# adobe/3D-FM-GAN

Measured on AMD Instinct MI355X. Metric: (photo,render) pairs/sec, higher is better.
Workload: dtype f32; 1 GPU; pairs1024: cfg4 shard: E_Tsr+E_W+E_W_Plus(18 styles) on 256^2 -> co-mod -> Generator(1024) forward, fp32, B=8/GPU; pairs_per_gpu=8, global_pairs=8, image_size=1024, parallelism=replicas x1 (batch-sharded, no collective), launch=eager, ranks=1, full=False

## Files before the change

3d-fm-gan_amd/csrc/modconv_fwd.hip:

```cpp
#include <type_traits>
#include "common.h"
#include <cstdio>
#include <cstdlib>

namespace {

typedef unsigned u32x2 __attribute__((ext_vector_type(2)));

template <int SIZE, typename RSRC>
__device__ __forceinline__ void dma_to_lds(RSRC rsrc, float* lds, unsigned voff, unsigned soff) {
#if defined(__HIP_DEVICE_COMPILE__)
  typedef __attribute__((address_space(3))) void* lds_void_ptr;
  __builtin_amdgcn_raw_ptr_buffer_load_lds(rsrc, (lds_void_ptr)lds, SIZE, voff, soff, 0, 0);
#endif
}

__device__ __forceinline__ const float* uniform_ptr(const float* q) {
  const unsigned long long v = (unsigned long long)q;
  const unsigned lo = __builtin_amdgcn_readfirstlane((unsigned)v), hi = __builtin_amdgcn_readfirstlane((unsigned)(v >> 32));
  return (const float*)(((unsigned long long)hi << 32) | lo);
}
__device__ __forceinline__ unsigned uniform_u32(unsigned v) { return __builtin_amdgcn_readfirstlane(v); }

struct MCParams {
  const float* in; const float* wt; const float* style; const float* demod; float* out;
  int batch, cin, cout, h, w, oh, ow;
  long long out_plane_stride; int out_row_stride;
  struct Seg {
    int m_off, n_off, gh, gw;
    int th, nb, tw_log2;
    int tiles_x, tiles_y, tiles_b;
    unsigned block_end;
    int wide;
  } seg[3];
  int nseg, o_tiles;
  int ksplit, cin_per_split;
  float* ws;
  const float* noise; const float* noise_weight; const float* bias;
  int noise_batch, fuse_act; float alpha, act_scale;
  const float* rgb_wmod;
  const float* rgb_bias; const float* rgb_skip; float* rgb_out;
  int rgb_c;
  int lds_buf_floats, lds_patch_floats;
  int lds_style_floats;
  int debug;
  unsigned long long* dbg_clock;
  int exp_flags;
};

#ifdef FMGAN_EXPERIMENTS
#define MC_DEBUG(p) ((p).debug)
#define MC_CLOCK(p) ((p).dbg_clock)
#define MC_FLAGS(p) ((p).exp_flags)
#else
#define MC_DEBUG(p) 0
#define MC_CLOCK(p) false
#define MC_FLAGS(p) 0
#endif

constexpr int MC_KC = 8;

__device__ __forceinline__ float mc_epilogue(float v, const MCParams& p, float nw, int b, int o, int pix) {
  if (p.demod) v *= p.demod[(long long)b * p.cout + o];
  if (p.fuse_act) {
    const float n = p.noise ? p.noise[(long long)(p.noise_batch == 1 ? 0 : b) * p.oh * p.ow + pix] : 0.f;
    const float bv = p.bias ? p.bias[o] : 0.f;
    v = __fadd_rn(__fadd_rn(v, __fmul_rn(nw, n)), bv);
    v = (v > 0.f ? v : v * p.alpha) * p.act_scale;
  }
  return v;
}

template <int MODE_, int RM_, int RNP_, int WM_, int WN_, int MINB_, int KC_, int PIPE_>
struct TileShape {
  static constexpr int MODE = MODE_, RM = RM_, RNP = RNP_, WM = WM_, WN = WN_, MINB = MINB_, KC = KC_, PIPE = PIPE_;
  static constexpr int BM = 32 * RM * WM, BN = 32 * RNP * WN;
};
struct Plain128x128Reg         : TileShape<   0,  2,   2,  2,  2,    2, MC_KC,    0> {};
struct Plain128x128DmaKc4      : TileShape<   0,  2,   2,  2,  2,    3,     4,    1> {};
struct Plain128x256DmaKc4      : TileShape<   0,  4,   2,  1,  4,    2,     4,    1> {};
struct Plain64x128Reg          : TileShape<   0,  2,   1,  1,  4,    3, MC_KC,    0> {};
struct Plain64x128Dma          : TileShape<   0,  2,   1,  1,  4,    3,     8,    1> {};
struct Plain64x256DmaKc4       : TileShape<   0,  2,   2,  1,  4,    3,     4,    1> {};
struct Plain32x128Reg          : TileShape<   0,  1,   1,  1,  4,    4, MC_KC,    0> {};
struct Plain32x128Dma          : TileShape<   0,  1,   1,  1,  4,    4,     8,    1> {};
struct Plain32x256DmaKc4R128   : TileShape<   0,  1,   2,  1,  4,    4,     4,    1> {};
struct Stride2x128x128Reg      : TileShape<   2,  2,   2,  2,  2,    2, MC_KC,    0> {};
struct Stride2x64x128Reg       : TileShape<   2,  2,   1,  1,  4,    2, MC_KC,    0> {};
struct Stride2x32x128Reg       : TileShape<   2,  1,   1,  1,  4,    2, MC_KC,    0> {};
struct Transposed64x128Reg     : TileShape<   1,  2,   1,  1,  4,    2, MC_KC,    0> {};
struct Transposed64x128Dma     : TileShape<   1,  2,   1,  1,  4,    2,     8,    1> {};
struct Transposed32x128Reg     : TileShape<   1,  1,   1,  1,  4,    3, MC_KC,    0> {};
struct Transposed32x128DmaR128 : TileShape<   1,  1,   1,  1,  4,    4,     8,    1> {};
#ifdef FMGAN_EXPERIMENTS
struct Plain32x256Dma          : TileShape<   0,  1,   2,  1,  4,    3,     8,    1> {};
struct Plain32x256DmaKc4R96    : TileShape<   0,  1,   2,  1,  4,    5,     4,    1> {};
struct Transposed32x256Dma     : TileShape<   1,  1,   2,  1,  4,    2,     8,    1> {};
struct Transposed32x128DmaR170 : TileShape<   1,  1,   1,  1,  4,    3,     8,    1> {};
#endif

template <class Tile, bool RGB>
__global__ __launch_bounds__(256, Tile::MINB) void modconv_mfma_f32(const MCParams p) {
  constexpr int MODE = Tile::MODE, RM = Tile::RM, RNP = Tile::RNP, WM = Tile::WM, WN = Tile::WN, KC = Tile::KC, PIPE = Tile::PIPE;
  static_assert(!RGB || MODE == 0, "the RGB epilogue belongs to the plain conv");
  static_assert(PIPE == 1 || KC == MC_KC, "the register pipeline is built for 8-channel chunks");
  constexpr int BM = Tile::BM;
  constexpr int NPH = MODE == 1 ? 4 : 1;
  static_assert(WM * WN == 4, "4 waves per block");
  extern __shared__ float smem[];
  float* Ws = smem;
  float* Xs = smem + KC * 9 * BM;

  const int tid = threadIdx.x, lane = tid & 63, wave = __builtin_amdgcn_readfirstlane(tid >> 6);
  const int wm = wave / WN, wn = wave % WN;
  const int l31 = lane & 31, khalf = lane >> 5;
  unsigned long long clk0 = 0, rt0 = 0;
  if (MC_CLOCK(p)) { clk0 = __builtin_readcyclecounter(); rt0 = wall_clock64(); }
  if (MC_FLAGS(p) & 1) __builtin_amdgcn_s_setprio(3);

  unsigned lb = xcd_remap(blockIdx.x, gridDim.x);
  int si = 0;
  while (si + 1 < p.nseg && lb >= p.seg[si].block_end) ++si;
  if (si > 0) lb -= p.seg[si - 1].block_end;
  const unsigned tapmask = (MODE == 1 && p.nseg == 3) ? (si == 0 ? 0x1C0u : (si == 1 ? 0x124u : 0x1FFu)) : 0x1FFu;
  const int seg_th = p.seg[si].th, seg_nb = p.seg[si].nb, tw_log2 = p.seg[si].tw_log2;
  const int seg_m_end = p.seg[si].m_off + p.seg[si].gh, seg_n_end = p.seg[si].n_off + p.seg[si].gw;
  constexpr int SP = MODE == 2 ? 2 : 1;
  constexpr int ORG = MODE == 2 ? 0 : 1;
  const bool wide = PIPE == 1 && SP == 1 && p.seg[si].wide != 0;
  const int XORG = wide ? 4 : ORG;
  const int TW = 1 << tw_log2, PWP = wide ? TW + 8 : SP * (TW - 1) + 3;
  const int o_tile = lb % p.o_tiles;
  unsigned pt = lb / p.o_tiles;
  const int tx_i = pt % p.seg[si].tiles_x; pt /= p.seg[si].tiles_x;
  const int ty_i = pt % p.seg[si].tiles_y;
  const int tb_i = pt / p.seg[si].tiles_y;
  const int ks = blockIdx.y;
  const int o0 = o_tile * BM, b0 = tb_i * seg_nb;
  const int x0 = p.seg[si].n_off + tx_i * TW, y0 = p.seg[si].m_off + ty_i * seg_th;
  const int PH = SP * (seg_th - 1) + 3;
  const int plane = PH * PWP;
  const int samp = KC * plane;

  int pbase[RNP], pos_b[RNP], pos_y[RNP], pos_x[RNP];
#pragma unroll
  for (int g = 0; g < RNP; ++g) {
    const int pos = (wn * RNP + g) * 32 + l31;
    const int tx = pos & (TW - 1), r = pos >> tw_log2;
    const int ty = r % seg_th, nbi = r / seg_th;
    pbase[g] = min(nbi, seg_nb - 1) * samp + SP * ty * PWP + SP * tx + (XORG - ORG);
    pos_b[g] = nbi < seg_nb ? b0 + nbi : p.batch; pos_y[g] = y0 + ty; pos_x[g] = x0 + tx;
  }

  f32x16 acc[RM][RNP][NPH];
#pragma unroll
  for (int a = 0; a < RM; ++a)
#pragma unroll
    for (int b = 0; b < RNP; ++b)
#pragma unroll
      for (int c = 0; c < NPH; ++c)
#pragma unroll
        for (int r = 0; r < 16; ++r) acc[a][b][c][r] = 0.f;

  const bool wvec = (p.cout & 3) == 0;
  const int i_begin = ks * p.cin_per_split;
  const int i_end = min(p.cin, i_begin + p.cin_per_split);
  const int hw = p.h * p.w;

  constexpr int BNP = 32 * RNP * WN;
  constexpr int NU = ((SP * (BNP / 32 - 1) + 3) * (SP * 31 + 3) + 255) / 256;
  constexpr int NWV = (KC * 9 * (BM / 4) + 255) / 256;
  const int spatial = seg_nb * plane;
  const float* in_b0 = uniform_ptr(p.in + (long long)b0 * p.cin * hw);
  const float* style_b0 = uniform_ptr(p.style + (long long)b0 * p.cin);
  const bool epi_lds = PIPE == 1 && seg_nb == 1 && p.ksplit == 1;
  float* Es = smem + 2 * p.lds_buf_floats;
  float epi_v = 0.f;
  if constexpr (PIPE == 1) {
    if (epi_lds && tid < 2 * BM) {
      const bool isd = tid >= BM;
      const int oc = min(o0 + (isd ? tid - BM : tid), p.cout - 1);
      epi_v = isd ? 1.f : 0.f;
      if (isd) { if (p.demod) epi_v = p.demod[(long long)min(b0, p.batch - 1) * p.cout + oc]; }
      else if (MODE == 0 && p.fuse_act && p.bias) epi_v = p.bias[oc];
    }
  }
  int gofs[NU], lofs[NU], sofs[NU]; bool inb[NU];
#pragma unroll
  for (int u = 0; u < NU; ++u) {
    const int q = tid + 256 * u;
    const int c = q % PWP;
    int t = q / PWP;
    const int r = t % PH, nbi = t / PH;
    const int b = b0 + nbi, y = SP * y0 + r - ORG, x = SP * x0 + c - ORG;
    inb[u] = q < spatial && b < p.batch && y >= 0 && y < p.h && x >= 0 && x < p.w;
    gofs[u] = inb[u] ? (nbi * p.cin * p.h + y) * p.w + x : 0;
    sofs[u] = nbi * p.cin;
    lofs[u] = q < spatial ? nbi * samp + r * PWP + c : -1;
  }
  float xv[NU][KC];
  f32x4 wv[NWV];
  constexpr long long PARK = 0xFFFFFFF0LL;
  const bool fastw = wvec && o0 + BM <= p.cout && (long long)p.cin * 9 * p.cout * 4 < PARK;
  const bool fastx = (long long)min(seg_nb, p.batch - b0) * p.cin * hw * 4 < PARK;
  const unsigned w_bytes = uniform_u32((unsigned)((long long)p.cin * 9 * p.cout * 4));
  const unsigned x_bytes = uniform_u32((unsigned)((long long)min(seg_nb, p.batch - b0) * p.cin * hw * 4));
  const auto rsrc_w = __builtin_amdgcn_make_buffer_rsrc(const_cast<float*>(p.wt), 0, w_bytes, 0x00020000);
  const auto rsrc_x = __builtin_amdgcn_make_buffer_rsrc(const_cast<float*>(in_b0), 0, x_bytes, 0x00020000);
  unsigned wofs[NWV], xofs[NU];
#pragma unroll
  for (int j = 0; j < NWV; ++j) {
    const int idx = tid + 256 * j;
    const int row = idx / (BM / 4), c4 = idx % (BM / 4);
    wofs[j] = idx < KC * 9 * (BM / 4) ? (unsigned)((row * p.cout + o0 + c4 * 4) * 4) : 0xFFFFFFF0u;
  }
#pragma unroll
  for (int u = 0; u < NU; ++u) xofs[u] = inb[u] ? (unsigned)gofs[u] * 4u : 0xFFFFFFF0u;
  auto issue = [&](int i0) {
    if (fastw && i0 + KC <= i_end) {
      const unsigned soff = (unsigned)(i0 * 9 * p.cout * 4);
#pragma unroll
      for (int j = 0; j < NWV; ++j) {
        const auto t = __builtin_amdgcn_raw_buffer_load_b128(rsrc_w, wofs[j], soff, 0);
        wv[j] = __builtin_bit_cast(f32x4, t);
      }
    } else {
#pragma unroll
      for (int j = 0; j < NWV; ++j) {
        const int idx = tid + 256 * j;
        const int row = idx / (BM / 4), c4 = idx % (BM / 4);
        const int i = i0 + row / 9, o = o0 + c4 * 4;
        f32x4 v = {0.f, 0.f, 0.f, 0.f};
        if (idx < KC * 9 * (BM / 4) && i < i_end) {
          const float* src = p.wt + ((long long)i * 9 + row % 9) * p.cout + o;
          if (wvec && o + 3 < p.cout) {
            v = *reinterpret_cast<const f32x4*>(src);
          } else {
            if (o + 0 < p.cout) v.x = src[0];
            if (o + 1 < p.cout) v.y = src[1];
            if (o + 2 < p.cout) v.z = src[2];
            if (o + 3 < p.cout) v.w = src[3];
          }
        }
        wv[j] = v;
      }
    }
    if (fastx && i0 + KC <= i_end) {
#pragma unroll
      for (int kc = 0; kc < KC; ++kc) {
        const unsigned soff = (unsigned)((i0 + kc) * hw * 4);
#pragma unroll
        for (int u = 0; u < NU; ++u)
          xv[u][kc] = __builtin_bit_cast(float, __builtin_amdgcn_raw_buffer_load_b32(rsrc_x, xofs[u], soff, 0));
      }
    } else {
#pragma unroll
      for (int u = 0; u < NU; ++u)
#pragma unroll
        for (int kc = 0; kc < KC; ++kc) {
          const int i = i0 + kc;
          xv[u][kc] = (inb[u] && i < i_end) ? in_b0[gofs[u] + i * hw] : 0.f;
        }
    }
  };
  auto commit = [&](int i0) {
#pragma unroll
    for (int j = 0; j < NWV; ++j) {
      const int idx = tid + 256 * j;
      if (idx < KC * 9 * (BM / 4)) *reinterpret_cast<f32x4*>(Ws + idx * 4) = wv[j];
    }
#pragma unroll
    for (int u = 0; u < NU; ++u)
      if (lofs[u] >= 0) {
        float sv[KC];
#pragma unroll
        for (int kc = 0; kc < KC; ++kc) sv[kc] = (inb[u] && i0 + kc < i_end) ? style_b0[sofs[u] + i0 + kc] : 0.f;
#pragma unroll
        for (int kc = 0; kc < KC; ++kc) Xs[lofs[u] + kc * plane] = xv[u][kc] * sv[kc];
      }
    for (int q = tid + 256 * NU; q < spatial; q += 256) {
      const int c = q % PWP;
      int t = q / PWP;
      const int r = t % PH, nbi = t / PH;
      const int b = b0 + nbi, y = SP * y0 + r - ORG, x = SP * x0 + c - ORG;
      const bool ok = b < p.batch && y >= 0 && y < p.h && x >= 0 && x < p.w;
      for (int kc = 0; kc < KC; ++kc) {
        const int i = i0 + kc;
        float v = 0.f;
        if (ok && i < i_end) {
          const long long ch = (long long)b * p.cin + i;
          v = p.in[(ch * p.h + y) * p.w + x] * p.style[ch];
        }
        Xs[nbi * samp + kc * plane + r * PWP + c] = v;
      }
    }
  };

  constexpr int NTA = MODE == 1 ? 9 : 3;
  constexpr int NTB = MODE == 1 ? 4 : 3;
  constexpr int NSTAGE = (KC / 2) * (MODE == 1 ? 1 : 3);
  struct Ops { float a[NTA][RM]; float b[NTB][RNP]; float s[RNP]; };
  const float* Wc = Ws;
  const float* Xc = Xs;
  const float* Sc = nullptr;
  int sbase[RNP];
#pragma unroll
  for (int g = 0; g < RNP; ++g) sbase[g] = (pbase[g] / samp) * KC;
  auto fetch = [&](Ops& o, int st) {
    const int kk = MODE == 1 ? st : st / 3, ky = MODE == 1 ? 0 : st % 3;
    const int kc = 2 * kk + khalf;
    const float* wrow = Wc + (kc * 9 + ky * 3) * BM + wm * 32 * RM + l31;
    const float* xrow = Xc + kc * plane;
#pragma unroll
    for (int t = 0; t < NTA; ++t)
#pragma unroll
      for (int m = 0; m < RM; ++m) o.a[t][m] = wrow[t * BM + m * 32];
    if constexpr (PIPE == 1) {
      if (MODE == 1 || ky == 0) {
#pragma unroll
        for (int g = 0; g < RNP; ++g) o.s[g] = Sc[sbase[g] + kc];
      }
    }
#pragma unroll
    for (int j = 0; j < NTB; ++j) {
      const int ro = MODE == 1 ? 1 - (j >> 1) : ky;
      const int co = MODE == 1 ? 1 - (j & 1) : j;
#pragma unroll
      for (int g = 0; g < RNP; ++g) o.b[j][g] = xrow[pbase[g] + ro * PWP + co];
    }
  };
  auto modulate = [&](Ops& o) {
    if constexpr (PIPE == 1) {
#pragma unroll
      for (int j = 0; j < NTB; ++j)
#pragma unroll
        for (int g = 0; g < RNP; ++g) o.b[j][g] *= o.s[g];
    }
  };
  auto mma = [&](const Ops& o, auto all_taps) {
    if constexpr (MODE != 1) {
#pragma unroll
      for (int t = 0; t < 3; ++t)
#pragma unroll
        for (int m = 0; m < RM; ++m)
#pragma unroll
          for (int g = 0; g < RNP; ++g)
            acc[m][g][0] = __builtin_amdgcn_mfma_f32_32x32x2f32(o.a[t][m], o.b[t][g], acc[m][g][0], 0, 0, 0);
    } else {
      constexpr int T[9][3] = {{0, 0, 0}, {2, 1, 0}, {6, 2, 0}, {8, 3, 0}, {1, 0, 1}, {7, 2, 1}, {3, 0, 2}, {5, 1, 2}, {4, 0, 3}};
#pragma unroll
      for (int q = 0; q < 9; ++q)
        if (decltype(all_taps)::value || (tapmask & (1u << T[q][0])))
#pragma unroll
          for (int m = 0; m < RM; ++m)
#pragma unroll
            for (int g = 0; g < RNP; ++g)
              acc[m][g][T[q][2]] =
                  __builtin_amdgcn_mfma_f32_32x32x2f32(o.a[T[q][0]][m], o.b[T[q][1]][g], acc[m][g][T[q][2]], 0, 0, 0);
    }
  };

  static_assert(NSTAGE % 2 == 0, "stages are processed in pairs");
  auto contract = [&](auto&& hook, auto all_taps) {
    Ops o0, o1;
    fetch(o0, 0);
#pragma unroll
    for (int st = 0; st < NSTAGE; st += 2) {
      __builtin_amdgcn_sched_barrier(0);
      hook(st);
      fetch(o1, st + 1);
      if constexpr (PIPE == 1 && MODE != 1) {
        if ((st + 1) % 3 != 0) {
#pragma unroll
          for (int g = 0; g < RNP; ++g) o1.s[g] = o0.s[g];
        }
      }
      __builtin_amdgcn_sched_barrier(0);
      modulate(o0);
      __builtin_amdgcn_s_setprio(1);
      mma(o0, all_taps);
      __builtin_amdgcn_s_setprio(0);
      __builtin_amdgcn_sched_barrier(0);
      hook(st + 1);
      if (st + 2 < NSTAGE) {
        fetch(o0, st + 2);
        if constexpr (PIPE == 1 && MODE != 1) {
          if ((st + 2) % 3 != 0) {
#pragma unroll
            for (int g = 0; g < RNP; ++g) o0.s[g] = o1.s[g];
          }
        }
      }
      __builtin_amdgcn_sched_barrier(0);
      modulate(o1);
      __builtin_amdgcn_s_setprio(1);
      mma(o1, all_taps);
      __builtin_amdgcn_s_setprio(0);
      __builtin_amdgcn_sched_barrier(0);
    }
  };

  unsigned long long clk1 = 0, clk2 = 0, clkw = 0, clke = 0, clkl = 0;
  if (MC_CLOCK(p)) clk1 = __builtin_readcyclecounter();
  if (MC_FLAGS(p) & 1) __builtin_amdgcn_s_setprio(0);
  if constexpr (PIPE == 0) {
    if (i_begin < i_end) issue(i_begin);
    for (int i0 = i_begin; i0 < i_end; i0 += KC) {
      const bool live = !(MC_DEBUG(p) & 1) || i0 == i_begin;
      if (!(MC_DEBUG(p) & 2)) __syncthreads();
      if (live) commit(i0);
      if (!(MC_DEBUG(p) & 2)) __syncthreads();
      __builtin_amdgcn_sched_barrier(0);
      if (live && i0 + KC < i_end) issue(i0 + KC);
      contract([](int) {}, std::false_type{});
    }
  } else {
    constexpr unsigned PARKED = 0xFFFFFFF0u;
    constexpr int WSZ = (KC * 9 * BM + 255) / 256 * 256;
    constexpr int WPIECES = WSZ / 256;
    constexpr int NWP = (WPIECES + 3) / 4;
    constexpr int NUP = ((KC * (SP * (BNP / 32 - 1) + 3) * (SP * 31 + 3) + 63) / 64 + 3) / 4;
    const int xs_total = seg_nb * samp;
    const int x_piece_floats = wide ? 256 : 64;
    const int x_pieces = (xs_total + x_piece_floats - 1) / x_piece_floats;
    const int s_pieces = (seg_nb * KC + 63) >> 6;
    const int bstride = p.lds_buf_floats;
    const bool fastc = fastw && fastx;
    const unsigned s_bytes = (unsigned)(min(seg_nb, p.batch - b0) * p.cin * 4);
    const auto rsrc_s = __builtin_amdgcn_make_buffer_rsrc(const_cast<float*>(style_b0), 0, s_bytes, 0x00020000);
    auto x_voff = [&](int e) -> unsigned {
      if (e >= xs_total) return PARKED;
      const int nbi = e / samp, rem = e - nbi * samp;
      const int kc = rem / plane, q = rem - kc * plane;
      const int r = q / PWP, c = q - r * PWP;
      const int b = b0 + nbi, y = SP * y0 + r - ORG, x = SP * x0 + c - XORG;
      const bool ok = b < p.batch && y >= 0 && y < p.h && x >= 0 && x < p.w;
      return ok ? (unsigned)(((nbi * p.cin + kc) * p.h + y) * p.w + x) * 4u : PARKED;
    };
    auto x_voff16 = [&](int g16) -> unsigned { return x_voff(4 * g16); };
    auto s_voff = [&](int e) -> unsigned {
      const int nbi = e / KC, kc = e - nbi * KC;
      return (nbi < seg_nb && b0 + nbi < p.batch) ? (unsigned)(nbi * p.cin + kc) * 4u : PARKED;
    };
    unsigned wvo[NWP], xvo[NUP];
#pragma unroll
    for (int j = 0; j < NWP; ++j) {
      const int idx = (4 * j + wave) * 64 + lane;
      const int row = idx / (BM / 4), c4 = idx % (BM / 4);
      wvo[j] = idx < KC * 9 * (BM / 4) ? (unsigned)((row * p.cout + o0 + c4 * 4) * 4) : PARKED;
    }
#pragma unroll
    for (int u = 0; u < NUP; ++u)
      xvo[u] = 4 * u + wave < x_pieces ? (wide ? x_voff16((4 * u + wave) * 64 + lane) : x_voff((4 * u + wave) * 64 + lane)) : PARKED;
    const unsigned svo = s_voff(wave * 64 + lane);

    constexpr int NPC = NWP + NUP + 1;
    constexpr int PER_STAGE = (NPC + NSTAGE - 1) / NSTAGE;
    auto dma_piece = [&](int k, int i0, int buf) {
      float* Wb = smem + buf * bstride;
      float* Xb = Wb + WSZ;
      const unsigned soff_x = (unsigned)(i0 * hw * 4);
      if (k < NWP) {
        if (4 * k + wave < WPIECES)
          dma_to_lds<16>(rsrc_w, Wb + (4 * k + wave) * 256, wvo[k < NWP ? k : 0], (unsigned)(i0 * 9 * p.cout * 4));
      } else if (k < NWP + NUP) {
        const int u = k - NWP;
        if (4 * u + wave < x_pieces) {
          if (wide) dma_to_lds<16>(rsrc_x, Xb + (4 * u + wave) * 256, xvo[(u >= 0 && u < NUP) ? u : 0], soff_x);
          else dma_to_lds<4>(rsrc_x, Xb + (4 * u + wave) * 64, xvo[(u >= 0 && u < NUP) ? u : 0], soff_x);
        }
      } else {
        float* Sb = Xb + p.lds_patch_floats;
        for (int pc = 4 * NUP + wave; pc < x_pieces; pc += 4) {
          if (wide) dma_to_lds<16>(rsrc_x, Xb + pc * 256, x_voff16(pc * 64 + lane), soff_x);
          else dma_to_lds<4>(rsrc_x, Xb + pc * 64, x_voff(pc * 64 + lane), soff_x);
        }
        if (wave < s_pieces)
          dma_to_lds<4>(rsrc_s, Sb + wave * 64, svo, (unsigned)(i0 * 4));
        for (int pc = 4 + wave; pc < s_pieces; pc += 4)
          dma_to_lds<4>(rsrc_s, Sb + pc * 64, s_voff(pc * 64 + lane), (unsigned)(i0 * 4));
      }
    };
    auto dma_ok = [&](int i0) { return fastc && i0 + KC <= i_end; };

    auto stage = [&](int i0, int buf) {
      float* Wb = smem + buf * bstride;
      float* Xb = Wb + WSZ;
      float* Sb = Xb + p.lds_patch_floats;
      if (dma_ok(i0)) {
#pragma unroll
        for (int k = 0; k < NPC; ++k) dma_piece(k, i0, buf);
      } else {
        for (int idx = tid; idx < KC * 9 * (BM / 4); idx += 256) {
          const int row = idx / (BM / 4), c4 = idx % (BM / 4);
          const int i = i0 + row / 9, o = o0 + c4 * 4;
          f32x4 v = {0.f, 0.f, 0.f, 0.f};
          if (i < i_end) {
            const float* src = p.wt + ((long long)i * 9 + row % 9) * p.cout + o;
            if (o + 0 < p.cout) v.x = src[0];
            if (o + 1 < p.cout) v.y = src[1];
            if (o + 2 < p.cout) v.z = src[2];
            if (o + 3 < p.cout) v.w = src[3];
          }
          *reinterpret_cast<f32x4*>(Wb + idx * 4) = v;
        }
        for (int e = tid; e < x_pieces * x_piece_floats; e += 256) {
          float v = 0.f;
          if (e < xs_total) {
            const int nbi = e / samp, rem = e - nbi * samp;
            const int kc = rem / plane, q = rem - kc * plane;
            const int r = q / PWP, c = q - r * PWP;
            const int b = b0 + nbi, y = SP * y0 + r - ORG, x = SP * x0 + c - XORG, i = i0 + kc;
            if (b < p.batch && y >= 0 && y < p.h && x >= 0 && x < p.w && i < i_end)
              v = p.in[(((long long)b * p.cin + i) * p.h + y) * p.w + x];
          }
          Xb[e] = v;
        }
        for (int e = tid; e < seg_nb * KC; e += 256) {
          const int nbi = e / KC, kc = e - nbi * KC;
          Sb[e] = (b0 + nbi < p.batch && i0 + kc < i_end) ? p.style[(long long)(b0 + nbi) * p.cin + i0 + kc] : 0.f;
        }
      }
    };

    const bool lean = fastc && MC_DEBUG(p) == 0 && i_begin < i_end && ((i_end - i_begin) % KC) == 0 && x_pieces <= 4 * NUP &&
                      s_pieces <= 4 && tapmask == 0x1FFu;
    const bool style_once = lean && seg_nb == 1 && p.lds_style_floats > 0;
    float* Ss = Es + 2 * BM;
    if (lean) {
      auto piece = [&](int k, int i0, int bufi) {
        float* Wb = smem + bufi * bstride;
        float* Xb = Wb + WSZ;
        if (k < NWP) {
          if (WPIECES % 4 == 0 || 4 * k + wave < WPIECES)
            dma_to_lds<16>(rsrc_w, Wb + (4 * k + wave) * 256, wvo[k < NWP ? k : 0], (unsigned)(i0 * 9 * p.cout * 4));
        } else if (k < NWP + NUP) {
          const int u = k - NWP;
          if (4 * u + wave < x_pieces) {
            if (wide) dma_to_lds<16>(rsrc_x, Xb + (4 * u + wave) * 256, xvo[(u >= 0 && u < NUP) ? u : 0], (unsigned)(i0 * hw * 4));
            else dma_to_lds<4>(rsrc_x, Xb + (4 * u + wave) * 64, xvo[(u >= 0 && u < NUP) ? u : 0], (unsigned)(i0 * hw * 4));
          }
        } else if (!style_once && wave < s_pieces) {
          dma_to_lds<4>(rsrc_s, Xb + p.lds_patch_floats + wave * 64, svo, (unsigned)(i0 * 4));
        }
      };
      float sty0 = 0.f, sty1 = 0.f;
      if (style_once) {
        const int n = i_end - i_begin;
        if (tid < n) sty0 = style_b0[i_begin + tid];
        if (tid + 256 < n) sty1 = style_b0[i_begin + tid + 256];
      }
#pragma unroll
      for (int k = 0; k < NPC; ++k) piece(k, i_begin, 0);
      if (epi_lds && tid < 2 * BM) Es[tid] = epi_v;
      if (style_once) {
        if (tid < p.lds_style_floats) Ss[tid] = sty0;
        if (tid + 256 < p.lds_style_floats) Ss[tid + 256] = sty1;
      }
      int bufl = 0;
      for (int i0 = i_begin; i0 < i_end; i0 += KC, bufl ^= 1) {
        const unsigned long long tw0 = MC_CLOCK(p) ? __builtin_readcyclecounter() : 0;
        __builtin_amdgcn_s_waitcnt(0);
        __builtin_amdgcn_s_barrier();
        __builtin_amdgcn_sched_barrier(0);
        if (MC_CLOCK(p)) clkw += __builtin_readcyclecounter() - tw0;
        const int i1 = i0 + KC;
        const bool more = i1 < i_end;
        Wc = smem + bufl * bstride;
        Xc = Wc + WSZ;
        Sc = style_once ? Ss + (i0 - i_begin) : Xc + p.lds_patch_floats;
        contract([&](int st) {
          if (more) {
#pragma unroll
            for (int q = 0; q < PER_STAGE; ++q)
              if (st * PER_STAGE + q < NPC) piece(st * PER_STAGE + q, i1, bufl ^ 1);
          }
        }, std::true_type{});
      }
    }
    if (!lean && i_begin < i_end) {
      stage(i_begin, 0);
      if (epi_lds && tid < 2 * BM) Es[tid] = epi_v;
    }
    int buf = 0;
    for (int i0 = lean ? i_end : i_begin; i0 < i_end; i0 += KC, buf ^= 1) {
      __builtin_amdgcn_s_waitcnt(0);
      if (!(MC_DEBUG(p) & 2)) __builtin_amdgcn_s_barrier();
      __builtin_amdgcn_sched_barrier(0);
      const int i1 = i0 + KC;
      const bool more = i1 < i_end && !(MC_DEBUG(p) & 1);
      const bool spread = more && dma_ok(i1) && !(MC_DEBUG(p) & 4);
      if (more && !spread) stage(i1, buf ^ 1);
      __builtin_amdgcn_sched_barrier(0);
      Wc = smem + buf * bstride;
      Xc = Wc + WSZ;
      Sc = Xc + p.lds_patch_floats;
      contract([&](int st) {
        if (spread) {
#pragma unroll
          for (int q = 0; q < PER_STAGE; ++q)
            if (st * PER_STAGE + q < NPC) dma_piece(st * PER_STAGE + q, i1, buf ^ 1);
        }
      }, std::false_type{});
    }
  }

  if (MC_CLOCK(p)) clk2 = __builtin_readcyclecounter();
  if (MC_FLAGS(p) & 1) __builtin_amdgcn_s_setprio(3);
  const bool partial = p.ksplit > 1;
  const bool actf = MODE == 0 && p.fuse_act && !partial;
  const bool use_demod = p.demod != nullptr && !partial;
  const float nw = (actf && p.noise && p.noise_weight) ? p.noise_weight[0] : 0.f;
  float* dstbase = partial ? p.ws + (long long)ks * p.batch * p.cout * p.oh * p.ow : p.out;
  const long long dps = partial ? (long long)p.oh * p.ow : p.out_plane_stride;
  const int drs = partial ? p.ow : p.out_row_stride;
  const int orow = o0 + wm * 32 * RM + 4 * khalf;
  bool vgs[RNP]; float nzs[RNP];
#pragma unroll
  for (int g = 0; g < RNP; ++g) {
    const int b = pos_b[g], bc = min(b, p.batch - 1);
    if constexpr (MODE != 1) {
      const int y = pos_y[g], x = pos_x[g];
      vgs[g] = b < p.batch && y < p.oh && x < p.ow;
      const int pix = vgs[g] ? y * p.ow + x : 0;
      nzs[g] = (actf && p.noise) ? __fmul_rn(nw, p.noise[(long long)(p.noise_batch == 1 ? 0 : bc) * p.oh * p.ow + pix]) : 0.f;
    } else {
      vgs[g] = b < p.batch && pos_y[g] < seg_m_end && pos_x[g] < seg_n_end;
      nzs[g] = 0.f;
    }
  }
  auto dpos_of = [&](int g) -> float* {
    const int bc = min(pos_b[g], p.batch - 1);
    const int sc = MODE == 1 ? 2 : 1;
    return dstbase + (long long)bc * p.cout * dps + (long long)(vgs[g] ? sc * pos_y[g] : 0) * drs + (vgs[g] ? sc * pos_x[g] : 0);
  };
  const long long slab = (long long)p.cout * dps * 4;
  bool bstore = dstbase != nullptr && o0 + BM <= p.cout && (long long)seg_nb * slab < 0xFFFFFFF0LL;
  if constexpr (MODE == 1) bstore = bstore && 2 * seg_m_end <= p.oh && 2 * seg_n_end <= p.ow;
  unsigned vofs[RNP];
  const float* obase = dstbase ? uniform_ptr(dstbase + (long long)b0 * p.cout * dps) : nullptr;
  const auto rsrc_o = __builtin_amdgcn_make_buffer_rsrc(const_cast<float*>(obase), 0,
      uniform_u32(bstore ? (unsigned)((long long)min(seg_nb, p.batch - b0) * slab) : 0u), 0x00020000);
#pragma unroll
  for (int g = 0; g < RNP; ++g) {
    const long long e = (long long)(pos_b[g] - b0) * p.cout * dps + (long long)(4 * khalf) * dps +
                        (long long)(MODE == 1 ? 2 * pos_y[g] : pos_y[g]) * drs + (MODE == 1 ? 2 * pos_x[g] : pos_x[g]);
    vofs[g] = (bstore && vgs[g]) ? (unsigned)(e * 4) : 0xFFFFFFF0u;
  }
  unsigned alpha_bits = __float_as_uint(p.alpha), ascale_bits = __float_as_uint(p.act_scale);
  asm volatile("" : "+s"(alpha_bits), "+s"(ascale_bits));
  const float alpha = __uint_as_float(alpha_bits), ascale = __uint_as_float(ascale_bits);
  const unsigned dps4 = uniform_u32((unsigned)(dps * 4)), drs4 = uniform_u32((unsigned)drs * 4u);
  if (MC_CLOCK(p)) clke = __builtin_readcyclecounter();
  auto rows = [&](auto act_c, auto bst_c) {
    constexpr bool ACT = decltype(act_c)::value, BST = decltype(bst_c)::value;
#pragma unroll
    for (int m = 0; m < RM; ++m) {
      float bias_m[16], dm_m[16];
      if (epi_lds) {
        const float* eb = Es + (orow - o0) + m * 32;
#pragma unroll
        for (int r = 0; r < 16; ++r) {
          bias_m[r] = ACT ? eb[(r & 3) + 8 * (r >> 2)] : 0.f;
          dm_m[r] = eb[BM + (r & 3) + 8 * (r >> 2)];
        }
      } else {
#pragma unroll
        for (int r = 0; r < 16; ++r) {
          const int oc = min(orow + m * 32 + (r & 3) + 8 * (r >> 2), p.cout - 1);
          bias_m[r] = (ACT && p.bias) ? p.bias[oc] : 0.f;
          dm_m[r] = 1.f;
        }
      }
      const unsigned so_m = (unsigned)(o0 + wm * 32 * RM + m * 32) * dps4;
#pragma unroll
      for (int g = 0; g < RNP; ++g) {
        const int bc = min(pos_b[g], p.batch - 1);
        if (!epi_lds && use_demod && (g == 0 || seg_nb > 1)) {
#pragma unroll
          for (int r = 0; r < 16; ++r)
            dm_m[r] = p.demod[(long long)bc * p.cout + min(orow + m * 32 + (r & 3) + 8 * (r >> 2), p.cout - 1)];
        }
        const bool vg = vgs[g];
        float* dpos = BST ? nullptr : dpos_of(g);
        if (MC_CLOCK(p) && m == 0 && g == 0) {
          __builtin_amdgcn_sched_barrier(0);
          __builtin_amdgcn_s_waitcnt(0);
          clkl = __builtin_readcyclecounter();
          __builtin_amdgcn_sched_barrier(0);
        }
        if constexpr (MODE != 1) {
          const float nz = nzs[g];
#pragma unroll
          for (int r = 0; r < 16; ++r) {
            const int o = orow + m * 32 + (r & 3) + 8 * (r >> 2);
            float v = acc[m][g][0][r] * dm_m[r];
            if constexpr (ACT) {
              v = __fadd_rn(__fadd_rn(v, nz), bias_m[r]);
              v = (v > 0.f ? v : v * alpha) * ascale;
            }
            if constexpr (BST) {
              if constexpr (RGB) acc[m][g][0][r] = vg ? v : 0.f;
              __builtin_amdgcn_raw_buffer_store_b32(__float_as_uint(v), rsrc_o, vofs[g], so_m + (unsigned)((r & 3) + 8 * (r >> 2)) * dps4, 0);
            } else {
              if constexpr (RGB) acc[m][g][0][r] = (vg && o < p.cout) ? v : 0.f;
              if ((!RGB || dstbase) && vg && o < p.cout) dpos[(long long)o * dps] = v;
            }
          }
        } else {
          const int X = 2 * pos_x[g], Y0 = 2 * pos_y[g];
          const bool pair = X + 1 < p.ow;
#pragma unroll
          for (int r = 0; r < 16; ++r) {
            const int o = orow + m * 32 + (r & 3) + 8 * (r >> 2);
            if constexpr (BST) {
#pragma unroll
              for (int py = 0; py < 2; ++py) {
                u32x2 t;
                t.x = __float_as_uint(acc[m][g][py * 2][r] * dm_m[r]);
                t.y = __float_as_uint(acc[m][g][py * 2 + 1][r] * dm_m[r]);
                __builtin_amdgcn_raw_buffer_store_b64(t, rsrc_o, vofs[g], so_m + (unsigned)((r & 3) + 8 * (r >> 2)) * dps4 + (unsigned)py * drs4, 0);
              }
            } else {
              if (!(vg && o < p.cout)) continue;
              float* dst = dpos + (long long)o * dps;
#pragma unroll
              for (int py = 0; py < 2; ++py) {
                if (Y0 + py >= p.oh) continue;
                const float v0 = acc[m][g][py * 2][r] * dm_m[r], v1 = acc[m][g][py * 2 + 1][r] * dm_m[r];
                if (pair) {
                  f32x2_u t; t.x = v0; t.y = v1;
                  *reinterpret_cast<f32x2_u*>(dst + (long long)py * drs) = t;
                } else {
                  dst[(long long)py * drs] = v0;
                }
              }
            }
          }
        }
      }
    }
  };
  if (bstore) {
    if (actf) rows(std::true_type{}, std::true_type{}); else rows(std::false_type{}, std::true_type{});
  } else {
    if (actf) rows(std::true_type{}, std::false_type{}); else rows(std::false_type{}, std::false_type{});
  }
  if (MC_CLOCK(p) && tid == 0 && (blockIdx.x & 63) == 0) {
    const unsigned long long clk3 = __builtin_readcyclecounter();
    atomicAdd(p.dbg_clock, clk3 - clk0);
    atomicAdd(p.dbg_clock + 1, wall_clock64() - rt0);
    atomicAdd(p.dbg_clock + 2, clk1 - clk0);
    atomicAdd(p.dbg_clock + 3, clk2 - clk1);
    atomicAdd(p.dbg_clock + 4, clk3 - clk2);
    atomicAdd(p.dbg_clock + 5, 1ULL);
    atomicAdd(p.dbg_clock + 8, clkl - clke);
    __builtin_amdgcn_s_waitcnt(0);
    atomicAdd(p.dbg_clock + 9, __builtin_readcyclecounter() - clk3);
    atomicAdd(p.dbg_clock + 7, clke - clk2);
    atomicAdd(p.dbg_clock + 6, clkw);
  }
  if constexpr (RGB) {
    float rs[RNP][3];
#pragma unroll
    for (int g = 0; g < RNP; ++g) rs[g][0] = rs[g][1] = rs[g][2] = 0.f;
    const float* wmod = p.rgb_wmod + (long long)min(b0, p.batch - 1) * 3 * p.cout;
#pragma unroll
    for (int m = 0; m < RM; ++m) {
      float rw[3][16];
#pragma unroll
      for (int r = 0; r < 16; ++r) {
        const int oc = min(orow + m * 32 + (r & 3) + 8 * (r >> 2), p.cout - 1);
#pragma unroll
        for (int c = 0; c < 3; ++c) rw[c][r] = wmod[c * p.cout + oc];
      }
#pragma unroll
      for (int g = 0; g < RNP; ++g)
#pragma unroll
        for (int r = 0; r < 16; ++r)
#pragma unroll
          for (int c = 0; c < 3; ++c) rs[g][c] = fmaf(acc[m][g][0][r], rw[c][r], rs[g][c]);
    }
#pragma unroll
    for (int g = 0; g < RNP; ++g)
#pragma unroll
      for (int c = 0; c < 3; ++c) rs[g][c] += __shfl_xor(rs[g][c], 32, 64);
    if constexpr (WM > 1) {
      static_assert(WM == 2, "two output-channel waves at most");
      __syncthreads();
      float* red = smem + ((wn * RNP) * 3) * 32;
      if (wm == 1 && khalf == 0)
#pragma unroll
        for (int g = 0; g < RNP; ++g)
#pragma unroll
          for (int c = 0; c < 3; ++c) red[(g * 3 + c) * 32 + l31] = rs[g][c];
      __syncthreads();
      if (wm == 0 && khalf == 0)
#pragma unroll
        for (int g = 0; g < RNP; ++g)
#pragma unroll
          for (int c = 0; c < 3; ++c) rs[g][c] += red[(g * 3 + c) * 32 + l31];
    }
    if (wm == 0 && khalf == 0) {
#pragma unroll
      for (int g = 0; g < RNP; ++g) {
        const int b = pos_b[g], y = pos_y[g], x = pos_x[g];
        if (b >= p.batch || y >= p.oh || x >= p.ow) continue;
#pragma unroll
        for (int c = 0; c < 3; ++c) {
          if (c >= p.rgb_c) continue;
          const long long off = (((long long)b * p.rgb_c + c) * p.oh + y) * p.ow + x;
          float v = rs[g][c];
          if (p.rgb_bias) v = __fadd_rn(v, p.rgb_bias[c]);
          if (p.rgb_skip) v = __fadd_rn(v, p.rgb_skip[off]);
          p.rgb_out[off] = v;
        }
      }
    }
  }
}

__global__ __launch_bounds__(256) void modconv_splitk_finish_f32(const MCParams p) {
  const float nw = (p.fuse_act && p.noise && p.noise_weight) ? p.noise_weight[0] : 0.f;
  const int hw = p.oh * p.ow;
  const long long total = (long long)p.batch * p.cout * hw;
  for (long long idx = (long long)blockIdx.x * blockDim.x + threadIdx.x; idx < total;
       idx += (long long)gridDim.x * blockDim.x) {
    float v = 0.f;
    for (int ks = 0; ks < p.ksplit; ++ks) v += p.ws[ks * total + idx];
    const int pix = (int)(idx % hw);
    const long long bo = idx / hw;
    p.out[bo * p.out_plane_stride + (long long)(pix / p.ow) * p.out_row_stride + pix % p.ow] =
        mc_epilogue(v, p, nw, (int)(bo / p.cout), (int)(bo % p.cout), pix);
  }
}

inline int pick_tw_log2(int gw, int gh) {
  if (gh <= 32 && gw <= 2) return gw <= 1 ? 0 : 1;
  return gw <= 4 ? 2 : (gw <= 8 ? 3 : (gw <= 16 ? 4 : 5));
}

inline bool mc_wide_patch() {
#ifdef FMGAN_EXPERIMENTS
  const char* e = getenv("FMGAN_MC_WIDE");
  return !(e && e[0] == '0');
#else
  return true;
#endif
}

inline long long plan_segment(MCParams::Seg& sg, int batch, int BN) {
  sg.tw_log2 = pick_tw_log2(sg.gw, sg.gh);
  const int TW = 1 << sg.tw_log2;
  const int rows_total = BN / TW;
  int th = rows_total, nb = 1;
  if (sg.gh < rows_total) {
    th = 1;
    while (th < sg.gh) th <<= 1;
    nb = rows_total / th;
  }
  sg.th = th; sg.nb = nb;
  sg.tiles_x = (sg.gw + TW - 1) / TW;
  sg.tiles_y = (sg.gh + th - 1) / th;
  sg.tiles_b = (batch + nb - 1) / nb;
  return (long long)sg.tiles_x * sg.tiles_y * sg.tiles_b;
}

constexpr size_t MC_LDS_LIMIT = 64 * 1024;
constexpr size_t MC_LDS_MAX = 160 * 1024;

struct MCPick {
  int cfg; char variant; int bm, bn, ksplit;
};

template <class Tile, bool FUSES_RGB>
int launch_tile(MCParams& p, hipStream_t s, bool plan_only) {
  constexpr int MODE = Tile::MODE, MINB = Tile::MINB, KC = Tile::KC, PIPE = Tile::PIPE, BM = Tile::BM, BN = Tile::BN;
  static_assert(!FUSES_RGB || MODE == 0, "the RGB epilogue belongs to the plain conv");
  if constexpr (!FUSES_RGB) { if (p.rgb_out) return FMGAN_EUNSUPPORTED; }
  constexpr int SP = MODE == 2 ? 2 : 1;
  p.o_tiles = (p.cout + BM - 1) / BM;
  long long blocks = 0;
  size_t patch = 0, nbmax = 1;
  auto patch_floats = [&](const MCParams::Seg& sg) {
    size_t f = (size_t)sg.nb * KC * (SP * (sg.th - 1) + 3) * (sg.wide ? (1 << sg.tw_log2) + 8 : SP * ((1 << sg.tw_log2) - 1) + 3);
    return sg.wide ? (f + 255) / 256 * 256 : f;
  };
  long long seg_blocks[3] = {0, 0, 0};
  int main_seg = 0;
  for (int i = 0; i < p.nseg; ++i) {
    seg_blocks[i] = plan_segment(p.seg[i], p.batch, BN);
    if (seg_blocks[i] > seg_blocks[main_seg]) main_seg = i;
    p.seg[i].wide = PIPE == 1 && SP == 1 && p.seg[i].tw_log2 == 5 && (p.seg[i].n_off & 3) == 0 && (p.w & 3) == 0 &&
                    (reinterpret_cast<uintptr_t>(p.in) & 15) == 0 && mc_wide_patch();
  }
  const size_t main_patch = patch_floats(p.seg[main_seg]);
  const bool cap_strips = seg_blocks[main_seg] * p.o_tiles >= 4LL * FMGAN_NUM_CU;
  for (int i = 0; i < p.nseg; ++i) {
    MCParams::Seg& sg = p.seg[i];
    while (cap_strips && i != main_seg && patch_floats(sg) > main_patch && (sg.nb > 1 || sg.th > 1)) {
      if (sg.nb > 1) sg.nb >>= 1; else sg.th >>= 1;
      sg.tiles_y = (sg.gh + sg.th - 1) / sg.th;
      sg.tiles_b = (p.batch + sg.nb - 1) / sg.nb;
      seg_blocks[i] = (long long)sg.tiles_x * sg.tiles_y * sg.tiles_b;
    }
    blocks += seg_blocks[i] * p.o_tiles;
    if (blocks > 0x7fffffffLL) return FMGAN_EOVERFLOW;
    sg.block_end = (unsigned)blocks;
    const int nb_live = sg.nb < p.batch ? sg.nb : p.batch;
    if ((long long)nb_live * p.cin * p.h * p.w >= (1LL << 31)) return FMGAN_EOVERFLOW;
    const size_t f = patch_floats(sg);
    if (f > patch) patch = f;
    if ((size_t)sg.nb > nbmax) nbmax = sg.nb;
  }
  size_t lds = sizeof(float) * ((size_t)KC * 9 * BM + patch);
  if constexpr (PIPE == 1) {
    if (p.cin_per_split % KC != 0) return 1;
    p.lds_patch_floats = (int)((patch + 63) / 64 * 64);
    p.lds_buf_floats = (KC * 9 * BM + 255) / 256 * 256 + p.lds_patch_floats + (int)((nbmax * KC + 63) / 64 * 64);
    p.lds_style_floats = (nbmax == 1 && p.cin_per_split <= 512) ? p.cin_per_split : 0;
    lds = sizeof(float) * (2 * (size_t)p.lds_buf_floats + 2 * BM + p.lds_style_floats);
    if (lds > (MINB == 1 ? MC_LDS_MAX : MC_LDS_LIMIT)) return 1;
    if (lds > MC_LDS_LIMIT && !plan_only) {
      static bool raised = false;
      if (!raised) {
        if (hipFuncSetAttribute(reinterpret_cast<const void*>(&modconv_mfma_f32<Tile, false>),
                                hipFuncAttributeMaxDynamicSharedMemorySize, (int)MC_LDS_MAX) != hipSuccess) {
          (void)hipGetLastError();
          return 1;
        }
        raised = true;
      }
    }
  }
  if constexpr (FUSES_RGB) {
    if (p.rgb_out) {
      if (p.o_tiles != 1 || p.ksplit != 1) return FMGAN_EUNSUPPORTED;
      if (nbmax > 1) return PIPE == 1 ? 1 : FMGAN_EUNSUPPORTED;
      if (plan_only) return FMGAN_OK;
      hipLaunchKernelGGL((modconv_mfma_f32<Tile, true>), dim3((unsigned)blocks, 1), dim3(256), lds, s, p);
      return fmgan_check_launch();
    }
  }
  if (plan_only) return FMGAN_OK;
  hipLaunchKernelGGL((modconv_mfma_f32<Tile, false>), dim3((unsigned)blocks, p.ksplit), dim3(256), lds, s, p);
  return fmgan_check_launch();
}

struct TileEntry {
  int mode, cfg;
  char variant;
  int BM, BN;
  bool fuses_rgb;
  int (*launch)(MCParams&, hipStream_t, bool plan_only);
};
template <class Tile, bool FUSES_RGB = false>
constexpr TileEntry tile_entry(int cfg, char variant) {
  return {Tile::MODE, cfg, variant, Tile::BM, Tile::BN, FUSES_RGB, &launch_tile<Tile, FUSES_RGB>};
}
#ifdef FMGAN_EXPERIMENTS
constexpr bool MC_EXP = true;
#else
constexpr bool MC_EXP = false;
#endif
constexpr TileEntry MC_TILES[] = {
    tile_entry<Plain128x256DmaKc4>(0, 'C'),
    tile_entry<Plain128x128DmaKc4, MC_EXP>(0, 'B'),
    tile_entry<Plain128x128Reg, true>(0, 'A'),
    tile_entry<Plain64x256DmaKc4>(1, 'C'),
    tile_entry<Plain64x128Dma, MC_EXP>(1, 'B'),
    tile_entry<Plain64x128Reg, true>(1, 'A'),
    tile_entry<Plain32x256DmaKc4R128, true>(2, 'E'),
    tile_entry<Plain32x128Dma, true>(2, 'B'),
    tile_entry<Plain32x128Reg, true>(2, 'A'),
#ifdef FMGAN_EXPERIMENTS
    tile_entry<Plain32x256Dma, true>(2, 'C'),
    tile_entry<Plain32x256DmaKc4R96, true>(2, 'D'),
#endif
    tile_entry<Transposed64x128Dma>(1, 'B'),
    tile_entry<Transposed64x128Reg>(1, 'A'),
    tile_entry<Transposed32x128DmaR128>(2, 'D'),
    tile_entry<Transposed32x128Reg>(2, 'A'),
#ifdef FMGAN_EXPERIMENTS
    tile_entry<Transposed32x256Dma>(1, 'C'),
    tile_entry<Transposed32x128DmaR170>(2, 'B'),
    tile_entry<Transposed32x256Dma>(2, 'C'),
#endif
    tile_entry<Stride2x128x128Reg>(0, 'A'),
    tile_entry<Stride2x64x128Reg>(1, 'A'),
    tile_entry<Stride2x32x128Reg>(2, 'A'),
};

inline const TileEntry* find_tile(int mode, int cfg, char variant) {
  for (const TileEntry& e : MC_TILES)
    if (e.mode == mode && e.cfg == cfg && e.variant == variant) return &e;
  return nullptr;
}

inline char mc_variant(int mode, int cfg) {
  char v = 'A';
  for (const TileEntry& e : MC_TILES)
    if (e.mode == mode && e.cfg == cfg) { v = e.variant; break; }
#ifdef FMGAN_EXPERIMENTS
  char name[32];
  snprintf(name, sizeof(name), "FMGAN_MC_V%d%d", mode, cfg);
  const char* e = getenv(name);
  if (e && e[0] >= 'A' && e[0] <= 'E') v = e[0];
#endif
  return v;
}

inline int pick_cfg(int mode, int cout, long long positions) {
  if (mode == 0) {
    if (positions <= 2048) return 2;
    return cout >= 96 ? 0 : (cout >= 48 ? 1 : 2);
  }
  if (mode == 2) return cout >= 96 ? 0 : (cout >= 48 ? 1 : 2);
  if (cout >= 192 && positions >= 4096) return 2;
  return cout >= 48 ? 1 : 2;
}

inline void model_tile_dims(int mode, int cfg, int& BM, int& BN) {
  (void)mode;
  const int bm[3] = {128, 64, 32};
  BM = bm[cfg]; BN = 128;
}

inline int model_blocks_per_cu(int mode, int cfg) {
  if (mode == 1) return cfg == 2 ? 3 : 2;
  return cfg == 0 ? 2 : (cfg == 1 ? (mode == 0 ? 3 : 2) : 4);
}

inline long long blocks_with(const MCParams& p, int BM, int BN) {
  long long blocks = 0;
  for (int i = 0; i < p.nseg; ++i) {
    MCParams::Seg sg = p.seg[i];
    blocks += plan_segment(sg, p.batch, BN);
  }
  return blocks * ((p.cout + BM - 1) / BM);
}

inline int launch_any(int mode, int cfg, MCParams& p, hipStream_t s, MCPick* pick = nullptr) {
  char v = mc_variant(mode, cfg);
  const TileEntry* e = nullptr;
  if (mode == 0 && v == 'C' && (e = find_tile(0, cfg, 'C')) != nullptr) {
    const bool small = p.ksplit > 1 || blocks_with(p, e->BM, e->BN) < 2LL * FMGAN_NUM_CU;
    if (cfg < 2 && (small || p.rgb_out)) v = (!p.rgb_out && (long long)p.batch * p.h * p.w >= 1536) ? 'B' : 'A';
    else if (cfg == 2 && small) v = 'B';
  }
  if (mode == 0 && (v == 'D' || v == 'E') && (e = find_tile(0, 2, v)) != nullptr) {
    const bool small = p.ksplit > 1 || blocks_with(p, e->BM, e->BN) < 2LL * FMGAN_NUM_CU;
    if (small) v = 'B';
  }
  int st = 1;
  if (v != 'A' && (e = find_tile(mode, cfg, v)) != nullptr) st = e->launch(p, s, pick != nullptr);
  if (st == 1) {
    e = find_tile(mode, cfg, 'A');
    st = e ? e->launch(p, s, pick != nullptr) : FMGAN_EUNSUPPORTED;
  }
  if (pick && st == FMGAN_OK) *pick = {cfg, e->variant, e->BM, e->BN, p.ksplit};
  return st;
}

inline void out_dims(int mode, int h, int w, int& oh, int& ow) {
  if (mode == 1) { oh = 2 * h + 1; ow = 2 * w + 1; }
  else if (mode == 2) { oh = (h - 3) / 2 + 1; ow = (w - 3) / 2 + 1; }
  else { oh = h; ow = w; }
}

inline long long count_blocks(int mode, int cfg, int batch, int cout, int h, int w) {
  int BM, BN;
  model_tile_dims(mode, cfg, BM, BN);
  if (mode == 2) out_dims(2, h, w, h, w);
  MCParams::Seg sg[3] = {{0, 0, h, w}, {h, 0, 1, w + 1}, {0, w, h, 1}};
  long long blocks = 0;
  for (int i = 0; i < (mode == 1 ? 3 : 1); ++i) blocks += plan_segment(sg[i], batch, BN);
  return blocks * ((cout + BM - 1) / BM);
}

inline int pick_ksplit(int mode, int batch, int cin, int cout, int h, int w) {
  int poh, pow_;
  out_dims(mode == 2 ? 2 : 0, h, w, poh, pow_);
  const int cfg = pick_cfg(mode, cout, (long long)batch * poh * pow_);
  const long long blocks = count_blocks(mode, cfg, batch, cout, h, w);
  const int chunks = (cin + MC_KC - 1) / MC_KC;
  const int slots = FMGAN_NUM_CU * model_blocks_per_cu(mode, cfg);
  if (blocks >= 4LL * slots || chunks < 4) return 1;
  int BM, BN;
  model_tile_dims(mode, cfg, BM, BN);
  const double mfma_per_chunk = (double)(BM / 32) * (BN / 32) * (mode == 1 ? 9 : 9) * (MC_KC / 2) / 4.0;
  const double t_chunk_us = mfma_per_chunk * 64.0 / 2360.0 * 2.0;
// ... 175 lines not shown
```

Before: 444.6 pairs/s.

## Fuse toRGB projection into modconv epilogue row loop with LDS-staged weights

Moves the fused toRGB 1x1 projection into the per-row epilogue so each activated output value is accumulated into the RGB sums as it is produced, rather than in a separate pass over the accumulators afterward. The modulated RGB weights, plus the bias and demod values for the non-pipelined variant, are staged once per block in extra LDS instead of being gathered per thread from global memory. This is meant to cut redundant global weight loads and register pressure in the RGB-fused layers. In exchange it uses more LDS, which can push some tile configurations past the limit and make them fall back to another path.

```diff
diff --git a/3d-fm-gan_amd/csrc/modconv_fwd.hip b/3d-fm-gan_amd/csrc/modconv_fwd.hip
--- a/3d-fm-gan_amd/csrc/modconv_fwd.hip
+++ b/3d-fm-gan_amd/csrc/modconv_fwd.hip
@@ -46,6 +46,7 @@
   int debug;
   unsigned long long* dbg_clock;
   int exp_flags;
+  int lds_rgb_off;
 };
 
 #ifdef FMGAN_EXPERIMENTS
@@ -173,10 +174,10 @@
   const int spatial = seg_nb * plane;
   const float* in_b0 = uniform_ptr(p.in + (long long)b0 * p.cin * hw);
   const float* style_b0 = uniform_ptr(p.style + (long long)b0 * p.cin);
-  const bool epi_lds = PIPE == 1 && seg_nb == 1 && p.ksplit == 1;
-  float* Es = smem + 2 * p.lds_buf_floats;
+  const bool epi_lds = (PIPE == 1 || RGB) && seg_nb == 1 && p.ksplit == 1;
+  float* Es = (PIPE == 0 && RGB) ? smem + p.lds_rgb_off + 4 * BM : smem + 2 * p.lds_buf_floats;
   float epi_v = 0.f;
-  if constexpr (PIPE == 1) {
+  if constexpr (PIPE == 1 || RGB) {
     if (epi_lds && tid < 2 * BM) {
       const bool isd = tid >= BM;
       const int oc = min(o0 + (isd ? tid - BM : tid), p.cout - 1);
@@ -185,6 +186,20 @@
       else if (MODE == 0 && p.fuse_act && p.bias) epi_v = p.bias[oc];
     }
   }
+  float* Rs = smem + p.lds_rgb_off;
+  f32x4 rgb_v = {0.f, 0.f, 0.f, 0.f};
+  if constexpr (RGB) {
+    if (tid < BM) {
+      const float* wmod = p.rgb_wmod + (long long)min(b0, p.batch - 1) * 3 * p.cout + min(o0 + tid, p.cout - 1);
+      rgb_v.x = wmod[0]; rgb_v.y = wmod[p.cout]; rgb_v.z = wmod[2 * p.cout];
+    }
+  }
+  auto put_rgb = [&]() {
+    if constexpr (RGB) {
+      if (tid < BM) *reinterpret_cast<f32x4*>(Rs + 4 * tid) = rgb_v;
+      if constexpr (PIPE == 0) { if (tid < 2 * BM) Es[tid] = epi_v; }
+    }
+  };
   int gofs[NU], lofs[NU], sofs[NU]; bool inb[NU];
 #pragma unroll
   for (int u = 0; u < NU; ++u) {
@@ -405,6 +420,7 @@
   if (MC_FLAGS(p) & 1) __builtin_amdgcn_s_setprio(0);
   if constexpr (PIPE == 0) {
     if (i_begin < i_end) issue(i_begin);
+    put_rgb();
     for (int i0 = i_begin; i0 < i_end; i0 += KC) {
       const bool live = !(MC_DEBUG(p) & 1) || i0 == i_begin;
       if (!(MC_DEBUG(p) & 2)) __syncthreads();
@@ -553,6 +569,7 @@
 #pragma unroll
       for (int k = 0; k < NPC; ++k) piece(k, i_begin, 0);
       if (epi_lds && tid < 2 * BM) Es[tid] = epi_v;
+      put_rgb();
       if (style_once) {
         if (tid < p.lds_style_floats) Ss[tid] = sty0;
         if (tid + 256 < p.lds_style_floats) Ss[tid + 256] = sty1;
@@ -582,6 +599,7 @@
       stage(i_begin, 0);
       if (epi_lds && tid < 2 * BM) Es[tid] = epi_v;
     }
+    if (!lean) put_rgb();
     int buf = 0;
     for (int i0 = lean ? i_end : i_begin; i0 < i_end; i0 += KC, buf ^= 1) {
       __builtin_amdgcn_s_waitcnt(0);
@@ -616,6 +634,7 @@
   const int drs = partial ? p.ow : p.out_row_stride;
   const int orow = o0 + wm * 32 * RM + 4 * khalf;
   bool vgs[RNP]; float nzs[RNP];
+  int rgb_pix[RNP];
 #pragma unroll
   for (int g = 0; g < RNP; ++g) {
     const int b = pos_b[g], bc = min(b, p.batch - 1);
@@ -623,10 +642,12 @@
       const int y = pos_y[g], x = pos_x[g];
       vgs[g] = b < p.batch && y < p.oh && x < p.ow;
       const int pix = vgs[g] ? y * p.ow + x : 0;
+      rgb_pix[g] = pix;
       nzs[g] = (actf && p.noise) ? __fmul_rn(nw, p.noise[(long long)(p.noise_batch == 1 ? 0 : bc) * p.oh * p.ow + pix]) : 0.f;
     } else {
       vgs[g] = b < p.batch && pos_y[g] < seg_m_end && pos_x[g] < seg_n_end;
       nzs[g] = 0.f;
+      rgb_pix[g] = 0;
     }
   }
   auto dpos_of = [&](int g) -> float* {
@@ -700,11 +721,9 @@
               v = (v > 0.f ? v : v * alpha) * ascale;
             }
             if constexpr (BST) {
-              if constexpr (RGB) acc[m][g][0][r] = vg ? v : 0.f;
               __builtin_amdgcn_raw_buffer_store_b32(__float_as_uint(v), rsrc_o, vofs[g], so_m + (unsigned)((r & 3) + 8 * (r >> 2)) * dps4, 0);
             } else {
-              if constexpr (RGB) acc[m][g][0][r] = (vg && o < p.cout) ? v : 0.f;
-              if ((!RGB || dstbase) && vg && o < p.cout) dpos[(long long)o * dps] = v;
+              if (vg && o < p.cout) dpos[(long long)o * dps] = v;
             }
           }
         } else {
@@ -741,7 +760,76 @@
       }
     }
   };
-  if (bstore) {
+  float rs[RNP][3];
+#pragma unroll
+  for (int g = 0; g < RNP; ++g) rs[g][0] = rs[g][1] = rs[g][2] = 0.f;
+  auto rows_rgb = [&](auto act_c, auto store_c) {
+    constexpr bool ACT = decltype(act_c)::value;
+    constexpr int STORE = decltype(store_c)::value;
+    float* dpos[RNP];
+#pragma unroll
+    for (int g = 0; g < RNP; ++g) dpos[g] = STORE == 0 ? dpos_of(g) : nullptr;
+#pragma unroll
+    for (int m = 0; m < RM; ++m) {
+      const float* eb = Es + (orow - o0) + m * 32;
+      const int rows_m = p.cout - (orow + m * 32);
+      const unsigned so_m = (unsigned)(o0 + wm * 32 * RM + m * 32) * dps4;
+      const float* rw_m = Rs + 4 * ((orow - o0) + m * 32);
+      if (MC_CLOCK(p) && m == 0) {
+        __builtin_amdgcn_sched_barrier(0);
+        __builtin_amdgcn_s_waitcnt(0);
+        clkl = __builtin_readcyclecounter();
+        __builtin_amdgcn_sched_barrier(0);
+      }
+#pragma unroll
+      for (int rq = 0; rq < 4; ++rq) {
+        __builtin_amdgcn_sched_barrier(0);
+        f32x4 rw[4];
+        float bias_q[4], dm_q[4];
+#pragma unroll
+        for (int j = 0; j < 4; ++j) {
+          rw[j] = *reinterpret_cast<const f32x4*>(rw_m + 4 * (8 * rq + j));
+          bias_q[j] = ACT ? eb[8 * rq + j] : 0.f;
+          dm_q[j] = eb[BM + 8 * rq + j];
+        }
+#pragma unroll
+        for (int g = 0; g < RNP; ++g) {
+#pragma unroll
+          for (int j = 0; j < 4; ++j) {
+            const int row = 8 * rq + j;
+            float v = acc[m][g][0][4 * rq + j] * dm_q[j];
+            if constexpr (ACT) {
+              v = __fadd_rn(__fadd_rn(v, nzs[g]), bias_q[j]);
+              v = (v > 0.f ? v : v * alpha) * ascale;
+            }
+            bool live = vgs[g];
+            if constexpr (STORE == 1) {
+              __builtin_amdgcn_raw_buffer_store_b32(__float_as_uint(v), rsrc_o, vofs[g], so_m + (unsigned)row * dps4, 0);
+            } else {
+              live = live && row < rows_m;
+              if constexpr (STORE == 0) { if (live) dpos[g][(long long)(orow + m * 32 + row) * dps] = v; }
+            }
+            const float a = live ? v : 0.f;
+            rs[g][0] = fmaf(a, rw[j].x, rs[g][0]);
+            rs[g][1] = fmaf(a, rw[j].y, rs[g][1]);
+            rs[g][2] = fmaf(a, rw[j].z, rs[g][2]);
+            if constexpr (STORE == 0) {
+              asm volatile("" : "+v"(rs[g][0]), "+v"(rs[g][1]), "+v"(rs[g][2]));
+            }
+          }
+        }
+      }
+    }
+  };
+  if constexpr (RGB) {
+    if (bstore) {
+      if (actf) rows_rgb(std::true_type{}, std::integral_constant<int, 1>{}); else rows_rgb(std::false_type{}, std::integral_constant<int, 1>{});
+    } else if (dstbase) {
+      if (actf) rows_rgb(std::true_type{}, std::integral_constant<int, 0>{}); else rows_rgb(std::false_type{}, std::integral_constant<int, 0>{});
+    } else {
+      if (actf) rows_rgb(std::true_type{}, std::integral_constant<int, 2>{}); else rows_rgb(std::false_type{}, std::integral_constant<int, 2>{});
+    }
+  } else if (bstore) {
     if (actf) rows(std::true_type{}, std::true_type{}); else rows(std::false_type{}, std::true_type{});
   } else {
     if (actf) rows(std::true_type{}, std::false_type{}); else rows(std::false_type{}, std::false_type{});
@@ -761,26 +849,6 @@
     atomicAdd(p.dbg_clock + 6, clkw);
   }
   if constexpr (RGB) {
-    float rs[RNP][3];
-#pragma unroll
-    for (int g = 0; g < RNP; ++g) rs[g][0] = rs[g][1] = rs[g][2] = 0.f;
-    const float* wmod = p.rgb_wmod + (long long)min(b0, p.batch - 1) * 3 * p.cout;
-#pragma unroll
-    for (int m = 0; m < RM; ++m) {
-      float rw[3][16];
-#pragma unroll
-      for (int r = 0; r < 16; ++r) {
-        const int oc = min(orow + m * 32 + (r & 3) + 8 * (r >> 2), p.cout - 1);
-#pragma unroll
-        for (int c = 0; c < 3; ++c) rw[c][r] = wmod[c * p.cout + oc];
-      }
-#pragma unroll
-      for (int g = 0; g < RNP; ++g)
-#pragma unroll
-        for (int r = 0; r < 16; ++r)
-#pragma unroll
-          for (int c = 0; c < 3; ++c) rs[g][c] = fmaf(acc[m][g][0][r], rw[c][r], rs[g][c]);
-    }
 #pragma unroll
     for (int g = 0; g < RNP; ++g)
 #pragma unroll
@@ -804,12 +872,11 @@
     if (wm == 0 && khalf == 0) {
 #pragma unroll
       for (int g = 0; g < RNP; ++g) {
-        const int b = pos_b[g], y = pos_y[g], x = pos_x[g];
-        if (b >= p.batch || y >= p.oh || x >= p.ow) continue;
+        if (!vgs[g]) continue;
 #pragma unroll
         for (int c = 0; c < 3; ++c) {
           if (c >= p.rgb_c) continue;
-          const long long off = (((long long)b * p.rgb_c + c) * p.oh + y) * p.ow + x;
+          const long long off = ((long long)b0 * p.rgb_c + c) * p.oh * p.ow + rgb_pix[g];
           float v = rs[g][c];
           if (p.rgb_bias) v = __fadd_rn(v, p.rgb_bias[c]);
           if (p.rgb_skip) v = __fadd_rn(v, p.rgb_skip[off]);
@@ -937,6 +1004,9 @@
     if (p.rgb_out) {
       if (p.o_tiles != 1 || p.ksplit != 1) return FMGAN_EUNSUPPORTED;
       if (nbmax > 1) return PIPE == 1 ? 1 : FMGAN_EUNSUPPORTED;
+      p.lds_rgb_off = (int)((lds / sizeof(float) + 3) / 4 * 4);
+      lds = sizeof(float) * ((size_t)p.lds_rgb_off + 4 * BM + (PIPE == 0 ? 2 * BM : 0));
+      if (lds > MC_LDS_LIMIT) return PIPE == 1 ? 1 : FMGAN_EUNSUPPORTED;
       if (plan_only) return FMGAN_OK;
       hipLaunchKernelGGL((modconv_mfma_f32<Tile, true>), dim3((unsigned)blocks, 1), dim3(256), lds, s, p);
       return fmgan_check_launch();
```

After: 448.7 pairs/s, median of 6. About the same (+0.9%).
